# JubSteven/POEM-v2

Hardware: AMD Instinct MI355X
Metric: samples/sec (multi-view frames) POEM-medium 8-view (higher is better)
Workload: dtype f32

## Files before the change

poem-v2_amd/csrc/decoder.cpp:

```cpp
#include "engine.h"

int build_anchor_tables(poem_handle_t h, Plan& p, hipStream_t s, bool at_create) {
  const poem_config_t& c = h->cfg;
  const int C = c.embed, Q = c.nquery;
  const bool ov = !at_create && h->overlap && h->bps_stream && h->knn_stream;
  hipStream_t sk = ov ? h->knn_stream : s;
  if (ov) {
    HIPCHK(hipEventRecord(h->ev_fork0, s));
    HIPCHK(hipStreamWaitEvent(sk, h->ev_fork0, 0));
  }
  const int bb0 = h->block_base(0);
  HIPCHK(poem_launch_canon_xyz(h->tmpl, p.canon_xyz, Q * 3, c.radius, sk));
  for (int k = 0; k < 2; ++k) {
    const int vb = bb0 + (k == 0 ? B_VS : B_VC);
    HIPCHK(poem_launch_vector_attention_tables(p.canon_xyz, h->anchor, h->anchor_idx, h->R(vb + 4), h->R(vb + 5),
                                               h->P(vb + 6), h->R(vb + 7), h->fused[0].w[5 + k], p.tab_g[k], p.tab_p[k],
                                               Q, C, sk));
  }
  if (ov) HIPCHK(hipEventRecord(h->ev_tab, sk));
  h->tables_pending = ov;
  return POEM_OK;
}

namespace {
// ... 212 lines not shown
      hidden = p.h_cross[i];
      ldh = C;
      if (tables && i == 0 && !anchor_from_y3) return anchor_rows_f3(i);
      return POEM_OK;
    }
    for (int a = 0; a < 2; ++a) {
      const int ab = bb + (a == 0 ? B_A1 : B_A2);
      float* hout = a == 0 ? p.h_attn : p.h_cross[i];
      const float* qptr = p.qeqp + C;
      int ldq = 2 * C;
      if (a == 1) {
        const int rc = gemm(hidden, ldh, ab + 0, ab + 1, nullptr, 0, p.qp, C, BQ, C, C, POEM_ACT_NONE);
        if (rc != POEM_OK) return rc;
        qptr = p.qp;
        ldq = C;
      }
      if (ov && a == 0) HIPCHK(hipStreamWaitEvent(s, h->ev_bps[i], 0));
      if (h->precision == POEM_PRECISION_SPLIT_F16X3_ALL) poem_cross_attention_split(h->kv_presplit[i] ? 2 : 1);
      if (h->precision == POEM_PRECISION_FP32 && merge_in_attention() && poem_cross_attention_merges(S, C, c.heads))
        HIPCHK(poem_launch_cross_attention_merged(qptr, ldq, Q, p.y1[i] + (size_t)(2 * a) * BSP * C, p.y1[i] + (size_t)(2 * a + 1) * BSP * C,
                                                  p.ctx, B, Q, S, C, c.heads, s));
      else
        HIPCHK(poem_launch_cross_attention_img(qptr, ldq, p.y1[i] + (size_t)(2 * a) * BSP * C, p.y1[i] + (size_t)(2 * a + 1) * BSP * C,
                                               p.ctx, B, Q, S, C, c.heads, p.attn_scratch, s));
      const int rc = gemm(p.ctx, C, ab + 6, ab + 7, hidden, ldh, p.att, C, BQ, C, C, POEM_ACT_NONE);
      if (rc != POEM_OK) return rc;
      HIPCHK(poem_launch_layernorm(p.att, h->R(ab + 8), h->R(ab + 9), hout, BQ, C, c.ln_eps, s));
      hidden = hout;
      ldh = C;
    }
    if (tables && i == 0) {
      HIPCHK(poem_launch_gemm(hidden, C, h->fused[i].w[2], h->fused[i].b[2], nullptr, 0, p.y3, 3 * C, BQ, C, C, POEM_ACT_NONE, s));
      return anchor_rows_f3(i);
    }
    HIPCHK(poem_launch_gemm_split(hidden, C, h->fused[i].w[2], h->fused[i].b[2], nullptr, 0, p.y3, 3 * C, BQ, 3 * C, C, POEM_ACT_NONE,
                                  3 * C, POEM_ACT_NONE, s));
    return POEM_OK;
  }

  int vector_self(int i) {
    const int vsb = h->block_base(i) + B_VS;
    const float* xyz = p.xyz[i];
    if (ov && i > 0 && !knn_waited[i]) HIPCHK(hipStreamWaitEvent(s, h->ev_knn[i], 0));
    const bool prof = prof_begin();
    const int kq = shared ? 32 : (h->knn_query ? h->knn_query : c.knn);
    if (h->precision != POEM_PRECISION_FP32) {
      if (kq != 32) return POEM_E_UNSUPPORTED;
      const auto& sw = h->split[2 * i];
      HIPCHK(poem_launch_vector_attention_split(xyz, xyz, anchor, idx_s, shared, p.y3, p.y3 + C, p.y3 + 2 * C, Q, h->R(vsb + 4),
                                                h->R(vsb + 5), sw.w[0], h->R(vsb + 7), sw.w[1], sw.w[2], sw.scales, p.rs, B, Q, C,
                                                3 * C, 3 * C, 3 * C, s));
    } else if (tables && i == 0) {
      if (ov && h->tables_pending) HIPCHK(hipStreamWaitEvent(s, h->ev_tab, 0));
      if (anchor_from_y3)
        HIPCHK(poem_launch_vector_attention_anchored(h->anchor_idx, p.y3, p.y3 + C, p.y3 + 2 * C, Q, h->P(vsb + 10), p.tab_g[0], p.tab_p[0],
                                                     p.rs, B, Q, C, 3 * C, 3 * C, 3 * C, s));
      else {
      if (ov) HIPCHK(hipStreamWaitEvent(s, h->ev_xyz[0], 0));
      HIPCHK(poem_launch_vector_attention_anchored(p.ident, p.y3, p.anch_kv[0], p.anch_kv[0] + C, 32, h->P(vsb + 10), p.tab_g[0],
                                                   p.tab_p[0], p.rs, B, Q, C, 3 * C, 2 * C, 2 * C, s));
      }
    } else if (!shared && p.idx_ld != 32) {
      HIPCHK(poem_launch_vector_attention_k(xyz, xyz, idx_s, kq, p.idx_ld, p.y3, p.y3 + C, p.y3 + 2 * C, Q, h->R(vsb + 4), h->R(vsb + 5),
                                            h->P(vsb + 6), h->R(vsb + 7), h->fused[i].w[5], h->R(vsb + 9), h->P(vsb + 10), h->R(vsb + 11),
                                            p.rs, B, Q, C, 3 * C, 3 * C, 3 * C, 1, s));
    } else {
      poem_vecattn_one_query_blocks(h->va_p1);
      poem_vecattn_valid_neighbours(kq);
      const hipError_t ve = poem_launch_vector_attention(xyz, xyz, anchor, idx_s, shared, p.y3, p.y3 + C, p.y3 + 2 * C, Q, h->R(vsb + 4),
                                                         h->R(vsb + 5), h->P(vsb + 6), h->R(vsb + 7), h->fused[i].w[5], h->R(vsb + 9),
                                                         h->P(vsb + 10), h->R(vsb + 11), p.rs, B, Q, C, 3 * C, 3 * C, 3 * C, 1, s);
      poem_vecattn_valid_neighbours(32);
      poem_vecattn_one_query_blocks(0);
      HIPCHK(ve);
    }
    if (const int rc = prof_end(prof, tables && i == 0 ? 1 : 0); rc != POEM_OK) return rc;
    if (chain) {
      ChainArgs cc = chain_args(1);
      cc.x = p.rs; cc.ldx = C;
      cc.w1 = (const float4*)h->P(vsb + 2); cc.b1 = h->R(vsb + 3); cc.res = hidden; cc.ldres = C; cc.res_mod = 0;
      cc.y1 = p.f_self[i]; cc.ldy1 = C;
      cc.w2 = (const float4*)h->fused[i].w[4]; cc.b2 = h->fused[i].b[4]; cc.n2 = 1; cc.y2 = p.qc; cc.ldy2 = C;
      HIPCHK(poem_launch_chain(&cc, C, s));
      return POEM_OK;
    }
    if (const int rc = gemm(p.rs, C, vsb + 2, vsb + 3, hidden, C, p.f_self[i], C, BQ, C, C, POEM_ACT_NONE); rc != POEM_OK) return rc;
    HIPCHK(poem_launch_gemm(p.f_self[i], C, h->fused[i].w[4], h->fused[i].b[4], nullptr, 0, p.qc, C, BQ, C, C, POEM_ACT_NONE, s));
    return POEM_OK;
  }

  int vector_cross(int i) {
    const int vcb = h->block_base(i) + B_VC;
    const float* xyz = p.xyz[i];
    if (ov && (wmask & 2) && i == 0 && defer_at() == 0)
      for (int k = 1; k < c.nblocks; ++k) {
        HIPCHK(hipStreamWaitEvent(s, h->ev_bps[k], 0));
        bps_waited[k] = true;
      }
    const bool prof = prof_begin();
    const int kc = shared ? 32 : c.knn;
    if (h->precision != POEM_PRECISION_FP32) {
      if (kc != 32) return POEM_E_UNSUPPORTED;
      const auto& sw = h->split[2 * i + 1];
      HIPCHK(poem_launch_vector_attention_split(xyz, pt_xyz_rows, anchor, idx_c, shared, p.qc, p.y1[i] + 4 * (size_t)BSP * C,
                                                p.y1[i] + 5 * (size_t)BSP * C, SP, h->R(vcb + 4), h->R(vcb + 5), sw.w[0],
                                                h->R(vcb + 7), sw.w[1], sw.w[2], sw.scales, p.rc, B, Q, C, C, C, C, s));
    } else if (tables && i == 0) {
      if (ov) HIPCHK(hipStreamWaitEvent(s, h->ev_xyz[0], 0));
      HIPCHK(poem_launch_vector_attention_anchored(p.ident, p.qc, p.anch_kv[1], p.anch_kv[1] + C, 32, h->P(vcb + 10), p.tab_g[1],
                                                   p.tab_p[1], p.rc, B, Q, C, C, 2 * C, 2 * C, s));
    } else if (!shared && p.idx_ld != 32) {
      HIPCHK(poem_launch_vector_attention_k(xyz, pt_xyz_rows, idx_c, kc, p.idx_ld, p.qc, p.y1[i] + 4 * (size_t)BSP * C, p.y1[i] + 5 * (size_t)BSP * C,
                                            SP, h->R(vcb + 4), h->R(vcb + 5), h->P(vcb + 6), h->R(vcb + 7), h->fused[i].w[6], h->R(vcb + 9),
                                            h->P(vcb + 10), h->R(vcb + 11), p.rc, B, Q, C, C, C, C, 1, s));
    } else {
      poem_vecattn_one_query_blocks(h->va_p1);
      poem_vecattn_valid_neighbours(kc);
      const hipError_t ve = poem_launch_vector_attention(xyz, pt_xyz_rows, anchor, idx_c, shared, p.qc, p.y1[i] + 4 * (size_t)BSP * C,
                                                         p.y1[i] + 5 * (size_t)BSP * C, SP, h->R(vcb + 4), h->R(vcb + 5), h->P(vcb + 6),
                                                         h->R(vcb + 7), h->fused[i].w[6], h->R(vcb + 9), h->P(vcb + 10), h->R(vcb + 11), p.rc, B,
                                                         Q, C, C, C, C, 1, s);
      poem_vecattn_valid_neighbours(32);
      poem_vecattn_one_query_blocks(0);
      HIPCHK(ve);
    }
    return prof_end(prof, tables && i == 0 ? 1 : 0);
  }

  int parametric_tail(int i) {
    const int bb = h->block_base(i);
    HIPCHK(poem_launch_q3_flatten(feats, h->R(bb + B_FLAT_W), h->R(bb + B_FLAT_B), p.q3t, B, Q, C, s));
    HIPCHK(poem_launch_narrow_linear(p.q3t, C, h->R(bb + B_MANO_W), h->R(bb + B_MANO_B), nullptr, p.par, B, C, 106, s));
    HIPCHK(poem_launch_rot6d_to_aa(p.par, pose_aa, betas, B, s));
    if (h->mano_table) HIPCHK(poem_launch_mano_lbs(pose_aa, betas, h->mano_table, p.mano_verts, p.mano_joints, B, h->mano_center, s));
    return POEM_OK;
  }

  int tail(int i, bool* done) {
    const int bb = h->block_base(i), vcb = bb + B_VC;
    const float* xyz = p.xyz[i];
    const bool last = i == c.nblocks - 1;
    const bool feats_dead = last && !c.parametric && !h->taps;
    *done = feats_dead;
    if (chain) {
      ChainArgs cd = chain_args(2);
      cd.x = p.rc; cd.ldx = C;
      cd.w1 = (const float4*)h->P(vcb + 2); cd.b1 = h->R(vcb + 3); cd.res = p.f_self[i]; cd.ldres = C; cd.res_mod = 0;
      cd.y1 = p.f_cross[i]; cd.ldy1 = C;
      cd.wf4 = (const float4*)h->fused[i].w[3]; cd.bf4 = h->fused[i].b[3];
      cd.wreg2 = h->R(bb + B_REG2_W); cd.breg2 = h->R(bb + B_REG2_B); cd.xyz_in = xyz; cd.xyz_out = p.xyz[i + 1];
      HIPCHK(poem_launch_chain(&cd, C, s));
      if (feats_dead) return POEM_OK;
      const bool early = ov && h->knn_early && !last;
      const bool d2_first = early && h->d2_first != 0;
      if (early && d2_first) HIPCHK(hipEventRecord(h->ev_xyz[i + 1], s));
      if (early && !d2_first)
        if (const int rc = neighbour_searches(i + 1); rc != POEM_OK) return rc;
      ChainArgs ce = chain_args(3);
      ce.x = p.f_cross[i]; ce.ldx = C;
      ce.wf4 = (const float4*)h->fused[i].w[3]; ce.bf4 = h->fused[i].b[3];
      ce.wout = (const float4*)h->P(bb + B_OUT_W); ce.bout = h->R(bb + B_OUT_B);
      ce.ln2_g = h->R(bb + B_LN_W); ce.ln2_b = h->R(bb + B_LN_B); ce.y3 = p.feats[i]; ce.ldy3 = C;
      if (!last) {
// ... 67 lines not shown
```

poem-v2_amd/csrc/engine.h:

```cpp
#pragma once
#include "../../include/poem_hip.h"
#include "launchers.h"

#include <hip/hip_runtime.h>

#include <algorithm>
#include <cstdio>
#include <cstdlib>
#include <cstring>
#include <map>
#include <string>
#include <vector>

extern thread_local int g_last_hip_error;

#define HIPCHK(expr)                                 \
  do {                                               \
    (void)hipGetLastError();                         \
    hipError_t e_ = (expr);                          \
    if (e_ != hipSuccess) {                          \
      g_last_hip_error = (int)e_;                    \
      return POEM_E_LAUNCH;                          \
    }                                                \
  } while (0)
// ... 48 lines not shown
  std::vector<SplitW> split;
  void* split_mem = nullptr;
  int precision = 0;
  bool kv_presplit[8] = {};
  const char* packed_base = nullptr;
  size_t packed_size = 0;
  char* native16 = nullptr;
  char* gemm_split = nullptr;
  float* gemm_scales = nullptr;
  bool taps = false;
  struct Tap { const void* p; int64_t elems; };
  std::map<std::string, Tap> tapmap;
  std::vector<hipEvent_t> prof_ev;
  int prof_used = 0;
  std::vector<char> prof_kind;
  bool prof_on = false;
  hipStream_t bps_stream = nullptr, knn_stream = nullptr;
  hipEvent_t ev_fork = nullptr, ev_join_bps = nullptr, ev_join_knn = nullptr, ev_tab = nullptr, ev_fork0 = nullptr;
  bool anchor_tables = true;
  bool chains = true;
  bool fused_sampling = true;
  bool tables_first = true;
  bool chain_combine = true;
  int xattn_merge = -1;
  bool knn_early = true;
  bool graphs = true;
  bool graph_broken = false;
  hipStream_t cap_stream = nullptr;
  int stream_device = 0;
  struct GraphEntry { std::vector<int64_t> key; hipGraphExec_t exec; uint64_t stamp; uint64_t shape; hipStream_t last_stream = nullptr; bool launched = false; };
  std::vector<GraphEntry> graph_cache;
  std::vector<std::vector<int64_t>> graph_seen;
  bool graph_eager = false;
  uint64_t graph_clock = 0;
  static constexpr size_t GRAPH_CAP = 12;
  int64_t graph_captures = 0, graph_instantiations = 0, graph_replays = 0, plain_forwards = 0, layout_uploads = 0;
  int small_batch = 3;
  int group_xcd = 1;
  int group_min_views = 0;
  const float* mano_table = nullptr;
  int mano_center = 9;
  int knn_query = 0;
  int knn_fma = 0;
  int chain_tile = 0;
  bool tables_cached = true;
  bool tables_pending = false;
  float* tab_mem = nullptr;
  float *c_canon_xyz = nullptr, *c_tab_g[2] = {}, *c_tab_p[2] = {};
  float* c_qeqp0 = nullptr;
  hipEvent_t ev_bps[8] = {}, ev_xyz[8] = {}, ev_knn[8] = {}, ev_def[8] = {};
  int bps_defer = 0;
  bool f1_split = true;
  int va_p1 = -1;
  int d2_first = 1;
  int wait_merge = -1;
  bool overlap = true;
  static constexpr int IDX_CAP = 32768;
  int32_t* idx_dev = nullptr;
  std::vector<int32_t> idx_host;
  int block_base(int b) const { return T_HEAD_COUNT + b * (cfg.parametric ? B_COUNT_PARAM : B_COUNT); }
  const float* R(int idx) const { return raw[idx]; }
  const void* P(int idx) const { return packed[idx]; }
};

struct Arena {
  char* base;
  size_t off = 0;
  explicit Arena(void* b) : base((char*)b) {}
  template <typename T>
  T* take(size_t n) {
    off = align_up(off, 256);
    T* p = base ? (T*)(base + off) : nullptr;
    off += n * sizeof(T);
    return p;
  }
};

struct Plan {
  int32_t *offs, *view_sample, *pe_index, *idx_self[8], *idx_cross[8];
  float *x, *uv, *g, *h1, *h2, *mm, *mh, *y, *bps_feat, *centre, *pt_xyz, *xyz[9];
  float *xt, *ptab, *q1;
  float *petr_f, *petr_h, *petr_tab;
  float *feats0, *qp, *ctx, *att, *h_attn, *y3, *rs, *qc, *rc, *y4, *ffo;
  float *y1[8];
  float *qeqp;
  float *h_cross[8], *f_self[8], *f_cross[8], *feats[8];
  float *q3t, *par, *attn_scratch, *g_pose, *g_betas;
  float *mano_verts, *mano_joints;
  float *canon_xyz, *tab_g[2], *tab_p[2];
  float *anch_x[2], *anch_kv[2], *qeqp0;
  int32_t* ident;
  float *feat_pad, *xyz_pad;
  int idx_ld;
  size_t bytes;
};

inline int padded_samples(const poem_config_t& c) { return (c.nsample + 31) / 32 * 32; }

inline int neighbour_ld(const poem_config_t& c, int knn_query) { return (c.knn > 32 || knn_query > 32) ? 64 : 32; }

Plan make_plan(const poem_config_t& c, int B, int BN, void* base, int idx_ld);
void register_taps(poem_handle_t h, const Plan& p, int B, int BN, bool sampling);

int poem_process_switches();
void poem_park_graph_exec(hipGraphExec_t e, uint64_t shape, int device, hipStream_t last_stream, bool launched);
hipGraphExec_t poem_reuse_graph_exec(hipGraph_t graph, uint64_t shape, int device);
// ... 5 lines not shown
```

poem-v2_amd/csrc/forward.cpp:

```cpp
#include "engine.h"

namespace {

struct SplitContext {
  bool set = false;
  explicit SplitContext(poem_handle_t h) {
    if (h->precision != POEM_PRECISION_SPLIT_F16X3_ALL) return;
    set = true;
    poem_gemm_split_context(h->packed_base, h->packed_size, h->gemm_split, h->gemm_scales);
    poem_cross_attention_split(1);
    const int dh = h->cfg.embed / h->cfg.heads;
    poem_gemm_split_images(dh == 32 || dh == 64);
  }
  ~SplitContext() {
    if (!set) return;
    poem_gemm_split_context(nullptr, 0, nullptr, nullptr);
    poem_cross_attention_split(0);
    poem_gemm_split_images(0);
  }
};

struct HeadRun {
  poem_handle_t h;
  const poem_config_t& c;
// ... 106 lines not shown
      SampleMergeArgs sm{};
      sm.xt = p.xt; sm.tab = (const float4*)p.ptab; sm.tabo = (const uint2*)(p.ptab + (size_t)plan_views * S * 4);
      sm.view_sample = p.view_sample; sm.offs = p.offs;
      sm.w0 = (const float4*)h->P(T_M00_W); sm.b0 = h->R(T_M00_B); sm.w1 = (const float4*)h->P(T_M02_W); sm.b1 = h->R(T_M02_B);
      sm.h2 = p.h2; sm.q1 = p.q1; sm.S = S; sm.hw = HW; sm.h2_tiled = 1;
      sm.views = plan_views; sm.B = B; sm.views_dev = p.offs + B;
      const bool group_ok = h->group_min_views >= 0 && (S / C) % 8 == 0;
      sm.group_min_views = group_ok ? (h->group_min_views > 0 ? h->group_min_views : 2 * poem_device_cu_count() / ((C / (C == 512 ? 32 : 64)) * (S / C / 8)))
                                    : 0x7fffffff;
      if (h->tables_first && h->tables_pending) HIPCHK(hipStreamWaitEvent(st, h->ev_tab, 0));
      MergeTailArgs mt{};
      mt.h2 = p.h2; mt.q1 = p.q1; mt.offs = p.offs;
      mt.w0 = (const float4*)h->P(T_M10_W); mt.b0 = h->R(T_M10_B); mt.w1 = (const float4*)h->P(T_M12_W); mt.b1 = h->R(T_M12_B);
      mt.out = p.bps_feat; mt.B = B; mt.S = S; mt.h2_tiled = 1;
      mt.group_min_views = sm.group_min_views; mt.views_dev = sm.views_dev; mt.views = sm.views;
      sm.xcd_order = h->group_xcd;
      if (group_ok && plan_views >= sm.group_min_views) {
        SampleGroupArgs sg{};
        sg.sm = sm; sg.w2 = mt.w0; sg.b2 = mt.b0; sg.w3 = mt.w1; sg.b3 = mt.b1; sg.out = p.bps_feat;
        HIPCHK(poem_launch_sample_group(&sg, C, st));
      }
      HIPCHK(poem_launch_sample_merge(&sm, C, st));
      HIPCHK(poem_launch_merge_tail(&mt, C, st));
      return POEM_OK;
    }
    auto gemm = [&](const float* X, int ldx, int wi, int bi, float* Y, int ldy, int M, int N, int K, int act) -> int {
      HIPCHK(poem_launch_gemm(X, ldx, h->P(wi), h->R(bi), nullptr, 0, Y, ldy, M, N, K, act, st));
      return POEM_OK;
    };
    HIPCHK(poem_launch_grid_sample(p.x, p.uv, p.g, BN, C, c.feat_h, c.feat_w, S, st));
    int rc = gemm(p.g, C, T_M00_W, T_M00_B, p.h1, C, BN * S, C, C, POEM_ACT_RELU);
    if (rc == POEM_OK) rc = gemm(p.h1, C, T_M02_W, T_M02_B, p.h2, C / 2, BN * S, C / 2, C, POEM_ACT_NONE);
    if (rc != POEM_OK) return rc;
    HIPCHK(poem_launch_merge_reduce(p.h2, p.offs, p.mm, B, S, C / 2, st));
    rc = gemm(p.mm, C / 2, T_M10_W, T_M10_B, p.mh, C / 2, BS, C / 2, C / 2, POEM_ACT_RELU);
    if (rc == POEM_OK) rc = gemm(p.mh, C / 2, T_M12_W, T_M12_B, p.y, C, BS, C, C / 2, POEM_ACT_NONE);
    if (rc != POEM_OK) return rc;
    HIPCHK(poem_launch_merge_finalize(p.g, p.y, p.offs, p.bps_feat, B, S, C, st));
    return POEM_OK;
  }

  int body(hipStream_t st, float* pose_dst, float* betas_dst) {
    if (const int rc = sampling(st); rc != POEM_OK) return rc;
    if (prof_fe) HIPCHK(hipEventRecord(h->prof_ev[2 * prof_slot + 1], st));
    if (!(h->anchor_tables && h->precision == POEM_PRECISION_FP32 && (h->small_batch & 1)))
      HIPCHK(poem_launch_broadcast(h->R(T_QEMB), p.feats0, (long)Q * C, B, st));
    return run_decoder(h, p, p.feats0, p.pt_xyz, p.bps_feat, B, pose_dst, betas_dst, st, true);
  }

  int replay(void* workspace, float* pose_aa, float* betas) {
    if (!h->graphs || h->graph_broken || h->prof_on || h->tables_pending || !h->cap_stream) return 0;
    const std::vector<int64_t> key = {B, plan_views, fused_fe ? -1 : BN, (int64_t)(uintptr_t)workspace, h->precision, h->anchor_tables, h->chains,
                                      h->fused_sampling, h->tables_first, h->chain_combine, h->knn_early, h->overlap, h->chain_tile,
                                      h->tables_cached, h->knn_fma, h->knn_query, h->taps, c.parametric, h->xattn_merge, h->small_batch, h->bps_defer, poem_process_switches(), h->f1_split, h->va_p1, h->group_min_views, h->group_xcd, h->d2_first, h->wait_merge,
                                      (int64_t)(uintptr_t)h->mano_table, h->mano_center};
    poem_handle_s::GraphEntry* hit = nullptr;
    for (auto& g : h->graph_cache)
      if (g.key == key) { hit = &g; break; }
    if (!hit) {
      if (!h->graph_eager) {
        bool seen = false;
        for (auto& k : h->graph_seen) seen = seen || k == key;
        if (!seen) {
          if (h->graph_seen.size() >= 64) h->graph_seen.erase(h->graph_seen.begin());
          h->graph_seen.push_back(key);
          return 0;
        }
      }
      hipGraph_t graph = nullptr;
      hipGraphExec_t exec = nullptr;
      POEM_TRACE("capture begin h=%p B=%d cached=%zu", (void*)h, B, h->graph_cache.size());
      bool ok = hipStreamBeginCapture(h->cap_stream, hipStreamCaptureModeRelaxed) == hipSuccess;
      if (ok) {
        const int rc = body(h->cap_stream, p.g_pose, p.g_betas);
        POEM_TRACE("capture body rc=%d", rc);
        const hipError_t e = hipStreamEndCapture(h->cap_stream, &graph);
        POEM_TRACE("capture end e=%d graph=%p", (int)e, (void*)graph);
        ok = rc == POEM_OK && e == hipSuccess && graph != nullptr;
      }
      ++h->graph_captures;
      if (ok) {
        exec = poem_reuse_graph_exec(graph, graph_shape_of(c, key), h->stream_device);
        if (!exec) {
          ok = hipGraphInstantiate(&exec, graph, nullptr, nullptr, 0) == hipSuccess;
          ++h->graph_instantiations;
        }
      }
      POEM_TRACE("instantiate ok=%d exec=%p", (int)ok, (void*)exec);
      if (graph) (void)hipGraphDestroy(graph);
      POEM_TRACE("graph destroyed");
      if (!ok) {
        (void)hipGetLastError();
        h->graph_broken = true;
        return 0;
      }
      if (h->graph_cache.size() >= poem_handle_s::GRAPH_CAP) {
        size_t lru = 0;
        for (size_t i = 1; i < h->graph_cache.size(); ++i)
          if (h->graph_cache[i].stamp < h->graph_cache[lru].stamp) lru = i;
        poem_park_graph_exec(h->graph_cache[lru].exec, h->graph_cache[lru].shape, h->stream_device, h->graph_cache[lru].last_stream,
                             h->graph_cache[lru].launched);
        h->graph_cache.erase(h->graph_cache.begin() + lru);
      }
      h->graph_cache.push_back({key, exec, 0, graph_shape_of(c, key), nullptr, false});
      hit = &h->graph_cache.back();
    }
    hit->stamp = ++h->graph_clock;
// ... 101 lines not shown
```

poem-v2_amd/csrc/handle.cpp:

```cpp
#include "engine.h"

#include <atomic>
thread_local int g_last_hip_error = 0;

static std::atomic<int> g_proc_switches{15};
int poem_process_switches() { return g_proc_switches.load(); }

#include <mutex>
namespace {
struct CaptureKit {
  hipStream_t cap = nullptr, bps = nullptr, knn = nullptr;
  hipEvent_t ev[5 + 32] = {};
};
std::mutex g_pool_mutex;
std::map<int, std::vector<CaptureKit>> g_kit_pool;
struct ParkedExec { hipGraphExec_t exec; uint64_t shape; int device; hipEvent_t done; };
std::vector<ParkedExec> g_parked_execs;
std::map<int, std::vector<hipEvent_t>> g_idle_done_events;
int64_t g_exec_reuses = 0, g_exec_update_failures = 0, g_exec_busy_skips = 0;

hipEvent_t done_event_locked(hipStream_t last_stream, bool launched, int device, bool* ok) {
  *ok = true;
  if (!launched) return nullptr;
  int cur = -1;
// ... 431 lines not shown
void poem_destroy(poem_handle_t h) {
  if (!h) return;
  POEM_TRACE("destroy h=%p graphs=%zu", (void*)h, h->graph_cache.size());
  for (auto e : h->prof_ev) (void)hipEventDestroy(e);
  if (h->tab_mem) (void)hipFree(h->tab_mem);
  if (h->split_mem) (void)hipFree(h->split_mem);
  if (h->gemm_split) (void)hipFree(h->gemm_split);
  if (h->native16) (void)hipFree(h->native16);
  if (h->gemm_scales) (void)hipFree(h->gemm_scales);
  park_execs(h);
  return_kit(h);
  delete h;
}

int poem_set_overlap(poem_handle_t h, int enable) {
  if (!h) return POEM_E_ARG;
  h->overlap = enable != 0;
  return POEM_OK;
}

int poem_set_chains(poem_handle_t h, int enable) {
  if (!h) return POEM_E_ARG;
  h->chains = enable != 0;
  return POEM_OK;
}

int poem_set_option(poem_handle_t h, const char* name, int value) {
  if (!h || !name) return POEM_E_ARG;
  const std::string k(name);
  if (k == "overlap") h->overlap = value != 0;
  else if (k == "anchor_tables") h->anchor_tables = value != 0;
  else if (k == "chains") h->chains = value != 0;
  else if (k == "knn_early") h->knn_early = value != 0;
  else if (k == "fused_sampling") h->fused_sampling = value != 0;
  else if (k == "chain_combine") h->chain_combine = value != 0;
  else if (k == "xattn_merge") { if (value < -1 || value > 1) return POEM_E_ARG; h->xattn_merge = value; }
  else if (k == "tables_first") h->tables_first = value != 0;
  else if (k == "tables_cached") h->tables_cached = value != 0;
  else if (k == "knn_fma") h->knn_fma = value != 0;
  else if (k == "knn_query") {
    if (value < 0 || value > 64 || value > h->cfg.nquery) return POEM_E_ARG;
    if (h->precision != POEM_PRECISION_FP32 && value != 0 && value != 32) return POEM_E_UNSUPPORTED;
    h->knn_query = value;
  }
  else if (k == "graphs") h->graphs = value != 0;
  else if (k == "graph_eager") h->graph_eager = value != 0;
  else if (k == "gemm_xcd_map") { poem_gemm_xcd_map(value != 0); g_proc_switches.fetch_and(~1); g_proc_switches.fetch_or(value ? 1 : 0); }
  else if (k == "f1_split") h->f1_split = value != 0;
  else if (k == "xattn_half") { poem_cross_attention_half(value != 0); g_proc_switches.fetch_and(~4); g_proc_switches.fetch_or(value ? 4 : 0); }
  else if (k == "xattn_tail") { poem_cross_attention_tail_halves(value != 0); g_proc_switches.fetch_and(~8); g_proc_switches.fetch_or(value ? 8 : 0); }
  else if (k == "wait_merge") { if (value < -1 || value > 7) return POEM_E_ARG; h->wait_merge = value; }
  else if (k == "d2_first") { if (value < 0 || value > 1) return POEM_E_ARG; h->d2_first = value; }
  else if (k == "va_p1") { if (value < -1 || value > 2) return POEM_E_ARG; h->va_p1 = value; }
  else if (k == "gemm_kslab") { poem_gemm_kslab(value != 0); g_proc_switches.fetch_and(~2); g_proc_switches.fetch_or(value ? 2 : 0); }
  else if (k == "small_batch") h->small_batch = value;
  else if (k == "group_xcd") h->group_xcd = value != 0;
  else if (k == "group_min_views") { if (value < -1) return POEM_E_ARG; h->group_min_views = value; }
  else if (k == "bps_defer") { if (value < 0 || value > 3) return POEM_E_ARG; h->bps_defer = value; }
  else if (k == "chain_tile") { if (value < 0 || value > 3) return POEM_E_ARG; h->chain_tile = value; }
  else return POEM_E_ARG;
  return POEM_OK;
}

int poem_graph_stats(poem_handle_t h, int64_t* out, int n) {
  if (!h || !out || n < 9) return POEM_E_ARG;
  out[0] = (int64_t)h->graph_cache.size();
  out[1] = h->graph_captures; out[2] = h->graph_instantiations; out[3] = h->graph_replays; out[4] = h->plain_forwards;
  out[5] = h->layout_uploads;
  std::lock_guard<std::mutex> lock(g_pool_mutex);
  out[6] = (int64_t)g_parked_execs.size(); out[7] = g_exec_reuses; out[8] = g_exec_update_failures;
  if (n >= 10) out[9] = g_exec_busy_skips;
  return POEM_OK;
}

int poem_attach_mano(poem_handle_t h, const void* table, int center_idx) {
  if (!h || center_idx < -1 || center_idx > 20) return POEM_E_ARG;
  if (table && !h->cfg.parametric) return POEM_E_UNSUPPORTED;
  h->mano_table = (const float*)table;
  h->mano_center = center_idx;
  return POEM_OK;
}

int poem_set_anchor_tables(poem_handle_t h, int enable) {
  if (!h) return POEM_E_ARG;
  h->anchor_tables = enable != 0;
  return POEM_OK;
}

int poem_set_precision(poem_handle_t h, int mode) {
  if (!h || mode < POEM_PRECISION_FP32 || mode > POEM_PRECISION_SPLIT_F16X3_ALL) return POEM_E_ARG;
  if (mode != POEM_PRECISION_FP32 && (!h->split_mem || !h->gemm_split)) return POEM_E_UNSUPPORTED;
  if (mode != POEM_PRECISION_FP32 && (h->cfg.knn != 32 || (h->knn_query && h->knn_query != 32)))
    return POEM_E_UNSUPPORTED;
  if (mode != POEM_PRECISION_FP32 && h->cfg.nsample % 32)
    return POEM_E_UNSUPPORTED;
  h->precision = mode;
  return POEM_OK;
}

int poem_enable_taps(poem_handle_t h, int enable) {
  if (!h) return POEM_E_ARG;
  h->taps = enable != 0;
  return POEM_OK;
}

int64_t poem_tap(poem_handle_t h, const char* name, void* dst, int64_t dst_elems, void* stream) {
// ... 58 lines not shown
```

poem-v2_amd/csrc/launchers.h:

```cpp
#pragma once
#include <hip/hip_runtime.h>

#include "../../include/poem_hip.h"
#include "chain.h"
#include "conv.h"
#include "loss.h"
#include "merge.h"

extern "C" {
hipError_t poem_launch_pack_linear(const float* w, int N, int K, void* out, hipStream_t s);
hipError_t poem_launch_gemm(const float* X, int ldx, const void* Wp, const float* bias, const float* R, int ldr,
                            float* Y, int ldy, int M, int N, int K, int act, hipStream_t s);
hipError_t poem_launch_gemm2(const float* X, int ldx, const void* Wp, const float* bias, const float* R, int ldr,
                             float* Y, int ldy, int M, int N, int K, int act, int in_pa, int out_pa, hipStream_t s);
hipError_t poem_launch_unpack_rows(const void* pa, int N, int K, float* out, hipStream_t s);
hipError_t poem_launch_layernorm(const float* x, const float* g, const float* b, float* y, int rows, int cols,
                                 float eps, hipStream_t s);
hipError_t poem_launch_narrow_linear(const float* x, int ldx, const float* w, const float* b, const float* base,
                                     float* out, int rows, int K, int N, hipStream_t s);
hipError_t poem_launch_sine_pe(float* out, int F, int H, int W, int max_views, int normalize, hipStream_t s);
hipError_t poem_launch_frustum_features(const float* intr, const float* extr, float* out, int views, int H, int W, int D, int lid,
                                        double depth_start, double depth_end, const double* position_range, int img0, int img1,
                                        hipStream_t s);
hipError_t poem_launch_conv1x1_ex(const float* feat, const void* Wp, const float* bias, const float* table, const int* pe_index,
// ... 35 lines not shown
hipError_t poem_launch_cross_attention_imgq(const float* q, int ldq, int q_batch_rows, const void* kimg, const void* vimg,
                                            float* ctx, int B, int NQ, int NK, int C, int heads, float* scratch, hipStream_t s);
int poem_chain_supported(int C);
int poem_chain_combines(int C, int heads, int chunks);
void poem_cross_attention_partials(int B, int NQ, int NK, int C, int heads, float* scratch, const void** part_o,
                                   const void** part_ml, int* chunks, float* kc2);
hipError_t poem_launch_chain(const ChainArgs* a, int C, hipStream_t s);
hipError_t poem_launch_native16(const void* packed, void* native, size_t bytes, hipStream_t s);
int poem_chain16_wants_native(int C);
hipError_t poem_launch_knn(const float* qxyz, const float* sxyz, int* idx, int B, int NQ, int NS, int fma, hipStream_t s);
hipError_t poem_launch_knn_k(const float* qxyz, const float* sxyz, int* idx, int B, int NQ, int NS, int K, int ld, int fma,
                             hipStream_t s);
hipError_t poem_launch_vector_attention(const float* query_xyz, const float* src_xyz, const float* anchor_xyz,
                                        const int* idx, int shared_idx, const float* q, const float* k, const float* v,
                                        int nsrc, const float* wd1, const float* bd1, const void* wd2, const float* bd2,
                                        const void* wg1, const float* bg1, const void* wg2, const float* bg2, float* out,
                                        int B, int Q, int C, int ldq, int ldk, int ldv, int composed, hipStream_t s);
hipError_t poem_launch_vector_attention_k(const float* query_xyz, const float* src_xyz, const int* idx, int K, int ld,
                                          const float* q, const float* k, const float* v, int nsrc, const float* wd1,
                                          const float* bd1, const void* wd2, const float* bd2, const void* wg1, const float* bg1,
                                          const void* wg2, const float* bg2, float* out, int B, int Q, int C, int ldq, int ldk,
                                          int ldv, int composed, hipStream_t s);
size_t poem_vector_attention_table_floats(int Q, int C);
hipError_t poem_launch_vector_attention_tables(const float* query_xyz, const float* anchor_xyz, const int* idx,
                                               const float* wd1, const float* bd1, const void* wd2, const float* bd2,
                                               const void* wg1d2, float* tab_g, float* tab_p, int Q, int C, hipStream_t s);
hipError_t poem_launch_vector_attention_anchored(const int* idx, const float* qg, const float* kg, const float* v, int nsrc,
                                                 const void* wg2, const float* tab_g, const float* tab_p, float* out, int B,
                                                 int Q, int C, int ldq, int ldk, int ldv, hipStream_t s);
hipError_t poem_launch_gather_anchor_rows(const float* src, int ld, const int* idx, int NS, float* dst, int B, int C,
                                          int* ident, hipStream_t s);
hipError_t poem_launch_pad_rows(const float* src, float* dst, int B, int S, int SP, int W, hipStream_t s);
hipError_t poem_launch_canon_xyz(const float* tmpl, float* out, int n, float radius, hipStream_t s);
hipError_t poem_launch_pack_split(const float* w, int C, void* img, float* scale_out, hipStream_t s);
hipError_t poem_launch_pack_split_tiles(const float* w, int N, int K, void* img, float* scales, int scale_stride, hipStream_t s);
void poem_gemm_split_context(const void* packed, size_t bytes, const void* split, const float* scales);
void poem_gemm_split_explicit(const void* img, const float* scales);
void poem_cross_attention_split(int on);
void poem_cross_attention_masked_form(int on);
void poem_cross_attention_half(int on);
void poem_cross_attention_tail_halves(int on);
int poem_cross_attention_merges(int NK, int C, int heads);
int poem_cross_attention_fits(int B, int NK, int C);
hipError_t poem_launch_cross_attention_merged_rm(const float* q, const float* k, const float* v, float* ctx, int B, int NQ, int NK,
                                                 int C, int heads, float* scratch, hipStream_t s);
hipError_t poem_launch_cross_attention_merged(const float* q, int ldq, int q_batch_rows, const void* kimg, const void* vimg, float* ctx,
                                              int B, int NQ, int NK, int C, int heads, hipStream_t s);
int poem_gemm_split_applies(const void* Wp, int M, int ldx, int K);
void poem_gemm_split_images(int on);
void poem_gemm_xcd_map(int on);
void poem_gemm_kslab(int on);
void poem_vecattn_one_query_blocks(int on);
void poem_vecattn_valid_neighbours(int k);
hipError_t poem_launch_vector_attention_split(const float* query_xyz, const float* src_xyz, const float* anchor_xyz,
                                              const int* idx, int shared_idx, const float* q, const float* k,
                                              const float* v, int nsrc, const float* wd1, const float* bd1,
                                              const void* wd2, const float* bd2, const void* wg1, const void* wg2,
                                              const float* scales, float* out, int B, int Q, int C, int ldq,
                                              int ldk, int ldv, hipStream_t s);
hipError_t poem_launch_dlt(const float* uv, const float* intr, const float* mat, const int* offs, float* out, int B, int J,
                           int invert, hipStream_t s);
hipError_t poem_launch_dlt_confidence(const float* uv, const float* conf, const float* intr, const float* mat,
                                      const int* offs, float* out, int* sel_count, int B, int J, int invert, int mode,
                                      double threshold, hipStream_t s);
hipError_t poem_launch_dlt_robust(const float* uv, const float* intr, const float* mat, const int* offs, float* out,
                                  unsigned char* inlier, int* count, float* resid, int B, int J, int invert,
                                  double inlier_px, int refine, hipStream_t s);
hipError_t poem_launch_pa_epe(const float* pred, const float* gt, float* out, int B, int P, hipStream_t s);
hipError_t poem_launch_pck_accumulate(const float* pred, const float* gt, int B, int P, double vmin, double vmax, int steps,
                                      unsigned int* counts, double* sum, unsigned int* n, float* dist_out, hipStream_t s);
hipError_t poem_launch_pa_align(const float* pred, const float* gt, float* aligned, double* transform, int B, int P, hipStream_t s);
size_t poem_nn_distance_slots(int B, int na, int nb);
hipError_t poem_launch_nn_distance(const float* a, int na, const float* b, int nb, float* dist_ab, float* dist_ba,
                                   const double* thr, int nthr, int* counts, double* sums, void* workspace, int B, hipStream_t s);
hipError_t poem_launch_mano_to_openpose(const float* jreg, const float* verts, float* joints, int B, int nverts,
                                        hipStream_t s);
hipError_t poem_launch_warp_affine(const unsigned char* src, const long long* src_off, const int* src_hw,
                                   const double* minv, const double* gain, float* out_f32, unsigned char* out_u8, int views,
                                   int OH, int OW, hipStream_t s);
hipError_t poem_launch_jpeg_reconstruct(const poem_jpeg_desc_t* descs, const int16_t* coef, long long coef_bytes,
                                        const long long* out_offsets, unsigned char* out, long long out_bytes, int n,
                                        long long total_blocks, long long total_quads, unsigned char* planes, hipStream_t s);
extern "C" size_t poem_jpeg_entropy_ws_bytes(int n, long long total_subs);
extern "C" hipError_t poem_launch_jpeg_entropy(poem_jpeg_desc_t* descs, const poem_jpeg_scan_t* scans, const poem_jpeg_huff_t* tables,
                                               long long table_count, const unsigned char* packed, long long packed_bytes, int n, int subseq,
                                               int wg_threads, long long total_subs, long long total_blocks, int16_t* coef,
                                               long long coef_bytes, int* status, void* workspace, hipStream_t s);
hipError_t poem_launch_heatmap_uv(const float* hmap, float* uv, int maps, int hh, int hw, float img_w, float img_h,
                                  hipStream_t s);
hipError_t poem_launch_heatmap_uv_conf(const float* hmap, float* uv, float* conf, int maps, int hh, int hw, float img_w,
                                       float img_h, hipStream_t s);
size_t poem_conv3x3_packed_floats(int Cout, int Cin);
hipError_t poem_launch_upcat_conv3x3(const float* a_half, int Ca, const float* b_full, int Cb, const void* wp, const float* scale,
                                     const float* shift, float* out, int views, int Cout, int H, int W, int relu, ConvMap omap,
                                     hipStream_t s);
hipError_t poem_launch_pack_conv3x3(const float* w, int Cout, int Cin, void* out, hipStream_t s);
hipError_t poem_launch_conv3x3(const float* in, const void* wp, const float* scale, const float* shift, const float* res,
                               float* out, int views, int Cin, int Cout, int H, int W, int stride, int relu, ConvMap omap,
                               hipStream_t s);
hipError_t poem_launch_conv3x3_ex(const float* in, const void* wp, const float* scale, const float* shift, const float* res,
                                  ConvMap rmap, int res_pre, float* out, int views, int Cin, int Cout, int H, int W, int stride,
                                  int relu, ConvMap omap, hipStream_t s);
size_t poem_conv1x1_packed_floats(int Cout, int Cin);
hipError_t poem_launch_pack_conv1x1(const float* w, int Cout, int Cin, void* out, hipStream_t s);
hipError_t poem_launch_conv1x1_nchw(const Conv1Args* a, hipStream_t s);
hipError_t poem_launch_hrnet_fuse(const FuseArgs* a, hipStream_t s);
// ... 58 lines not shown
```

poem-v2_amd/csrc/vecattn.hip:

```cpp
#include "common.h"
#ifndef POEM_VA_XCD_SAMPLES
#define POEM_VA_XCD_SAMPLES 1
#endif
#include <algorithm>
#include <cstdlib>

#ifdef POEM_VA_DBG
__device__ long long va_dbg[64 * 4 * 8];
#define VA_STAMP(k) do { if (item >= 6000 && item < 6064 && lane == 0) va_dbg[((item - 6000) * 4 + wv) * 8 + (k)] = clock64(); } while (0)
#else
#define VA_STAMP(k) do { } while (0)
#endif

struct VecAttnArgs {
  const float* query_xyz;
  const float* src_xyz;
  const float* anchor_xyz;
  const int* idx;
  int shared_idx;
  const float* q;
  const float* k;
  const float* v;
  int NS;
  const float* wd1;
// ... 422 lines not shown
#pragma unroll
      for (int i = 0; i < 16; ++i) pt[i] = COMP ? pos[tp][p][i] : scr[mfma_row(i, h) * 33 + j];
      f32x16& a = acc[tp][p];
      if (MASK) {
#pragma unroll
        for (int i = 0; i < 16; ++i)
          if (mfma_row(i, h) >= A.kvalid) a[i] = -INFINITY;
      }
      if (WIDE) {
#pragma unroll
        for (int i = 0; i < 16; ++i)
          if (32 * ch + mfma_row(i, h) >= A.kvalid) a[i] = -INFINITY;
      }
      float mx = fmaxf(fmaxf(a[0], a[1]), a[2]);
#pragma unroll
      for (int i = 3; i < 15; i += 2) mx = fmaxf(fmaxf(mx, a[i]), a[i + 1]);
      mx = half_max(fmaxf(mx, a[15]));
      const float nb = -mx * k2;
      const f32x2 k2v = {k2, k2}, nbv = {nb, nb};
      f32x2 sum2 = {0.f, 0.f}, res2 = {0.f, 0.f};
      asm volatile("s_waitcnt lgkmcnt(0)" ::: "memory");
#pragma unroll
      for (int i = 0; i < 16; i += 2) {
        f32x2 e = __builtin_elementwise_fma(f32x2{a[i], a[i + 1]}, k2v, nbv);
        e[0] = __builtin_amdgcn_exp2f(e[0]);
        e[1] = __builtin_amdgcn_exp2f(e[1]);
        const f32x2 val = f32x2{vg[i], vg[i + 1]} + f32x2{pt[i], pt[i + 1]};
        sum2 += e;
        res2 = __builtin_elementwise_fma(e, val, res2);
      }
      const float sum = half_sum(sum2[0] + sum2[1]);
      const float res = half_sum(res2[0] + res2[1]);
      if (WIDE) {
        if (ch == 0) {
          wmx[q] = mx; wsum[q] = sum; wres[q] = res;
        } else {
          const float m = fmaxf(wmx[q], mx), nm = -m * k2;
          const float so = __builtin_amdgcn_exp2f(__builtin_fmaf(wmx[q], k2, nm)), sn = __builtin_amdgcn_exp2f(__builtin_fmaf(mx, k2, nm));
          wsum[q] = __builtin_fmaf(wsum[q], so, sum * sn);
          wres[q] = __builtin_fmaf(wres[q], so, res * sn);
          wmx[q] = m;
        }
        if (ch == nch - 1 && h == 0 && i0 + p < A.Q) A.out[((size_t)b * A.Q + i0 + p) * C + cch] = wres[q] * __builtin_amdgcn_rcpf(wsum[q]);
      } else if (h == 0 && i0 + p < A.Q) A.out[((size_t)b * A.Q + i0 + p) * C + cch] = res * __builtin_amdgcn_rcpf(sum);
    }
  }
  if constexpr (WIDE)
    if (++ch < nch) goto va_chunk;
#undef VA_GATHER
  VA_STAMP(7);
  }
}

template <int C, int P, int NW, int MINW, bool COMP, int MODE = 0>
static hipError_t launch_va_t(const VecAttnArgs& a, hipStream_t s) {
  const int groups = (a.Q + P - 1) / P;
  size_t lds = (size_t)C * 32 * P * 4 + P * 32 * 3 * 4 + 2 * P * 32 * 4 + (size_t)P * C * 4;
#ifdef POEM_VA_DBG
  if (const char* e = getenv("POEM_VA_LDSPAD")) lds += atoi(e);
#endif
  auto kern = vecattn_kernel<C, P, NW, MINW, COMP, MODE>;
  static std::atomic<unsigned long long> optin{0};
  if (hipError_t e = poem_optin_lds(reinterpret_cast<const void*>(kern), lds, optin); e != hipSuccess) return e;
  unsigned grid = (unsigned)(a.B * groups);
  if (a.stagger > 0) {
    grid = std::min(grid, (unsigned)(2 * poem_device_cus()));
  }
  hipLaunchKernelGGL(kern, dim3(grid), dim3(NW * 64), lds, s, a);
  return hipGetLastError();
}

template <int C, int P, int NW, int MINW>
static hipError_t launch_va(const VecAttnArgs& a, hipStream_t s, int mode = 0) {
  if (mode == 4) return a.composed ? launch_va_t<C, P, NW, MINW, true, 4>(a, s) : launch_va_t<C, P, NW, MINW, false, 4>(a, s);
  if (mode == 1) return launch_va_t<C, P, NW, MINW, true, 1>(a, s);
  if (mode == 2) return launch_va_t<C, P, NW, MINW, true, 2>(a, s);
  if (mode == 3) return a.composed ? launch_va_t<C, P, NW, MINW, true, 3>(a, s) : hipErrorInvalidValue;
  return a.composed ? launch_va_t<C, P, NW, MINW, true>(a, s) : launch_va_t<C, P, NW, MINW, false>(a, s);
}

static thread_local int g_va_kvalid = 32;
extern "C" void poem_vecattn_valid_neighbours(int k) { g_va_kvalid = k; }

static thread_local int g_va_p1 = 0;
extern "C" void poem_vecattn_one_query_blocks(int on) { g_va_p1 = on; }

static int va_group_size(int C) { return C == 128 ? 4 : (C >= 512 ? 1 : 2); }

static hipError_t dispatch_va(const VecAttnArgs& a, int C, hipStream_t s, int mode) {
  if (mode != 1 && (unsigned long long)a.NS * a.ldv * 4 + (unsigned long long)C * 4 > (1ull << 31)) return hipErrorInvalidValue;
  if (mode == 4 && (a.kvalid < 1 || a.kvalid > 64 || a.ldidx < a.kvalid || a.shared_idx || a.anchor_xyz)) return hipErrorInvalidValue;
  if (mode == 0 && a.kvalid != 32) {
    if (a.kvalid < 1 || a.kvalid > 32) return hipErrorInvalidValue;
    mode = 3;
  }
  switch (C) {
    case 32: return launch_va<32, 2, 1, 1>(a, s, mode);
    case 64: return launch_va<64, 2, 2, 1>(a, s, mode);
    case 128: return launch_va<128, 4, 4, 2>(a, s, mode);
    case 256: {
      const int g_va_p1 = ::g_va_p1 >= 0 ? ::g_va_p1 : ((long)a.B * a.Q <= 16L * poem_device_cus() ? 1 : 0);
      if (mode == 0 && g_va_p1 == 1 && a.composed) return launch_va_t<256, 1, 4, 3, true>(a, s);
      if (mode == 0 && g_va_p1 == 2 && a.composed) return launch_va_t<256, 1, 4, 2, true>(a, s);
      return launch_va<256, 2, 4, 2>(a, s, mode);
    }
    case 512: return launch_va<512, 1, 4, 2>(a, s, mode);
    case 1024: return launch_va<1024, 1, 8, 2>(a, s, mode);
    default: return hipErrorInvalidValue;
  }
}

extern "C" size_t poem_vector_attention_table_floats(int Q, int C) {
  const int P = va_group_size(C);
  return (size_t)((Q + P - 1) / P) * P * 32 * C;
}

extern "C" hipError_t poem_launch_vector_attention_tables(const float* query_xyz, const float* anchor_xyz, const int* idx,
                                                          const float* wd1, const float* bd1, const void* wd2,
                                                          const float* bd2, const void* wg1d2, float* tab_g,
                                                          float* tab_p, int Q, int C, hipStream_t s) {
  VecAttnArgs a{query_xyz, nullptr, anchor_xyz, idx, 1, nullptr, nullptr, nullptr, 1, wd1, bd1, (const float4*)wd2, bd2,
                (const float4*)wg1d2, nullptr, nullptr, nullptr, nullptr, 1, Q, 0, 0, 0, 0, 1, (float4*)tab_g, (float4*)tab_p, 32, 32};
  return dispatch_va(a, C, s, 1);
}

extern "C" hipError_t poem_launch_vector_attention_anchored(const int* idx, const float* qg, const float* kg,
                                                            const float* v, int nsrc, const void* wg2,
                                                            const float* tab_g, const float* tab_p, float* out, int B,
                                                            int Q, int C, int ldq, int ldk, int ldv, hipStream_t s) {
// ... 43 lines not shown
```

Baseline: 1470.

## Add persistent walk kernel for anchored vector attention reusing position tables

After: 1476 (median of 6 runs). No clear change (+0.4%).

```diff
diff --git a/poem-v2_amd/csrc/decoder.cpp b/poem-v2_amd/csrc/decoder.cpp
--- a/poem-v2_amd/csrc/decoder.cpp
+++ b/poem-v2_amd/csrc/decoder.cpp
@@ -288,14 +288,15 @@
                                                 3 * C, 3 * C, 3 * C, s));
     } else if (tables && i == 0) {
       if (ov && h->tables_pending) HIPCHK(hipStreamWaitEvent(s, h->ev_tab, 0));
-      if (anchor_from_y3)
-        HIPCHK(poem_launch_vector_attention_anchored(h->anchor_idx, p.y3, p.y3 + C, p.y3 + 2 * C, Q, h->P(vsb + 10), p.tab_g[0], p.tab_p[0],
-                                                     p.rs, B, Q, C, 3 * C, 3 * C, 3 * C, s));
-      else {
-      if (ov) HIPCHK(hipStreamWaitEvent(s, h->ev_xyz[0], 0));
-      HIPCHK(poem_launch_vector_attention_anchored(p.ident, p.y3, p.anch_kv[0], p.anch_kv[0] + C, 32, h->P(vsb + 10), p.tab_g[0],
-                                                   p.tab_p[0], p.rs, B, Q, C, 3 * C, 2 * C, 2 * C, s));
-      }
+      if (!anchor_from_y3 && ov) HIPCHK(hipStreamWaitEvent(s, h->ev_xyz[0], 0));
+      poem_vecattn_anchored_walk(h->va_anchor_walk);
+      const hipError_t ve = anchor_from_y3
+          ? poem_launch_vector_attention_anchored(h->anchor_idx, p.y3, p.y3 + C, p.y3 + 2 * C, Q, h->P(vsb + 10), p.tab_g[0], p.tab_p[0],
+                                                  p.rs, B, Q, C, 3 * C, 3 * C, 3 * C, s)
+          : poem_launch_vector_attention_anchored(p.ident, p.y3, p.anch_kv[0], p.anch_kv[0] + C, 32, h->P(vsb + 10), p.tab_g[0],
+                                                  p.tab_p[0], p.rs, B, Q, C, 3 * C, 2 * C, 2 * C, s);
+      poem_vecattn_anchored_walk(0);
+      HIPCHK(ve);
     } else if (!shared && p.idx_ld != 32) {
       HIPCHK(poem_launch_vector_attention_k(xyz, xyz, idx_s, kq, p.idx_ld, p.y3, p.y3 + C, p.y3 + 2 * C, Q, h->R(vsb + 4), h->R(vsb + 5),
                                             h->P(vsb + 6), h->R(vsb + 7), h->fused[i].w[5], h->R(vsb + 9), h->P(vsb + 10), h->R(vsb + 11),
@@ -343,8 +344,11 @@
                                                 h->R(vcb + 7), sw.w[1], sw.w[2], sw.scales, p.rc, B, Q, C, C, C, C, s));
     } else if (tables && i == 0) {
       if (ov) HIPCHK(hipStreamWaitEvent(s, h->ev_xyz[0], 0));
-      HIPCHK(poem_launch_vector_attention_anchored(p.ident, p.qc, p.anch_kv[1], p.anch_kv[1] + C, 32, h->P(vcb + 10), p.tab_g[1],
-                                                   p.tab_p[1], p.rc, B, Q, C, C, 2 * C, 2 * C, s));
+      poem_vecattn_anchored_walk(h->va_anchor_walk);
+      const hipError_t ve = poem_launch_vector_attention_anchored(p.ident, p.qc, p.anch_kv[1], p.anch_kv[1] + C, 32, h->P(vcb + 10), p.tab_g[1],
+                                                                  p.tab_p[1], p.rc, B, Q, C, C, 2 * C, 2 * C, s);
+      poem_vecattn_anchored_walk(0);
+      HIPCHK(ve);
     } else if (!shared && p.idx_ld != 32) {
       HIPCHK(poem_launch_vector_attention_k(xyz, pt_xyz_rows, idx_c, kc, p.idx_ld, p.qc, p.y1[i] + 4 * (size_t)BSP * C, p.y1[i] + 5 * (size_t)BSP * C,
                                             SP, h->R(vcb + 4), h->R(vcb + 5), h->P(vcb + 6), h->R(vcb + 7), h->fused[i].w[6], h->R(vcb + 9),
diff --git a/poem-v2_amd/csrc/engine.h b/poem-v2_amd/csrc/engine.h
--- a/poem-v2_amd/csrc/engine.h
+++ b/poem-v2_amd/csrc/engine.h
@@ -124,6 +124,7 @@
   int bps_defer = 0;
   bool f1_split = true;
   int va_p1 = -1;
+  int va_anchor_walk = -1;
   int d2_first = 1;
   int wait_merge = -1;
   bool overlap = true;
diff --git a/poem-v2_amd/csrc/forward.cpp b/poem-v2_amd/csrc/forward.cpp
--- a/poem-v2_amd/csrc/forward.cpp
+++ b/poem-v2_amd/csrc/forward.cpp
@@ -182,7 +182,7 @@
     if (!h->graphs || h->graph_broken || h->prof_on || h->tables_pending || !h->cap_stream) return 0;
     const std::vector<int64_t> key = {B, plan_views, fused_fe ? -1 : BN, (int64_t)(uintptr_t)workspace, h->precision, h->anchor_tables, h->chains,
                                       h->fused_sampling, h->tables_first, h->chain_combine, h->knn_early, h->overlap, h->chain_tile,
-                                      h->tables_cached, h->knn_fma, h->knn_query, h->taps, c.parametric, h->xattn_merge, h->small_batch, h->bps_defer, poem_process_switches(), h->f1_split, h->va_p1, h->group_min_views, h->group_xcd, h->d2_first, h->wait_merge,
+                                      h->tables_cached, h->knn_fma, h->knn_query, h->taps, c.parametric, h->xattn_merge, h->small_batch, h->bps_defer, poem_process_switches(), h->f1_split, h->va_p1, h->va_anchor_walk, h->group_min_views, h->group_xcd, h->d2_first, h->wait_merge,
                                       (int64_t)(uintptr_t)h->mano_table, h->mano_center};
     poem_handle_s::GraphEntry* hit = nullptr;
     for (auto& g : h->graph_cache)
diff --git a/poem-v2_amd/csrc/handle.cpp b/poem-v2_amd/csrc/handle.cpp
--- a/poem-v2_amd/csrc/handle.cpp
+++ b/poem-v2_amd/csrc/handle.cpp
@@ -507,6 +507,7 @@
   else if (k == "wait_merge") { if (value < -1 || value > 7) return POEM_E_ARG; h->wait_merge = value; }
   else if (k == "d2_first") { if (value < 0 || value > 1) return POEM_E_ARG; h->d2_first = value; }
   else if (k == "va_p1") { if (value < -1 || value > 2) return POEM_E_ARG; h->va_p1 = value; }
+  else if (k == "va_anchor_walk") { if (value < -1 || value > 65536) return POEM_E_ARG; h->va_anchor_walk = value; }
   else if (k == "gemm_kslab") { poem_gemm_kslab(value != 0); g_proc_switches.fetch_and(~2); g_proc_switches.fetch_or(value ? 2 : 0); }
   else if (k == "small_batch") h->small_batch = value;
   else if (k == "group_xcd") h->group_xcd = value != 0;
diff --git a/poem-v2_amd/csrc/launchers.h b/poem-v2_amd/csrc/launchers.h
--- a/poem-v2_amd/csrc/launchers.h
+++ b/poem-v2_amd/csrc/launchers.h
@@ -111,6 +111,7 @@
 void poem_gemm_kslab(int on);
 void poem_vecattn_one_query_blocks(int on);
 void poem_vecattn_valid_neighbours(int k);
+void poem_vecattn_anchored_walk(int blocks);
 hipError_t poem_launch_vector_attention_split(const float* query_xyz, const float* src_xyz, const float* anchor_xyz,
                                               const int* idx, int shared_idx, const float* q, const float* k,
                                               const float* v, int nsrc, const float* wd1, const float* bd1,
diff --git a/poem-v2_amd/csrc/vecattn.hip b/poem-v2_amd/csrc/vecattn.hip
--- a/poem-v2_amd/csrc/vecattn.hip
+++ b/poem-v2_amd/csrc/vecattn.hip
@@ -498,6 +498,173 @@
   }
 }
 
+template <int C, int P, int NW, int MINW, int GT>
+__global__ __launch_bounds__(NW * 64, MINW) void vecattn_walk_kernel(VecAttnArgs A) {
+  constexpr int NTILE = C / 32;
+  constexpr int TPW = C / 32 / NW;
+  constexpr int XS = 32 * P;
+  constexpr int NT = NW * 64;
+  static_assert(GT >= 0 && GT <= TPW, "resident tab_g tiles: at most the wave's own");
+  extern __shared__ __attribute__((aligned(16))) float smem[];
+  float* X = smem;
+  int* voffs = reinterpret_cast<int*>(smem + C * XS + P * 32 * 3) + P * 32;
+  float* qs = reinterpret_cast<float*>(voffs + P * 32);
+
+  const int tid = threadIdx.x, lane = tid & 63, wv = tid >> 6, j = lane & 31, h = lane >> 5;
+  const int groups = (A.Q + P - 1) / P;
+  const int total = A.B * groups;
+  const float inv_sqrt_c = 1.0f / sqrtf((float)C);
+
+  const int nblk = (int)gridDim.x;
+  int slot = (int)blockIdx.x;
+  if ((nblk & 7) == 0) slot = (slot & 7) * (nblk >> 3) + (slot >> 3);
+  const int base = total / nblk, rem = total % nblk;
+  int item = slot * base + min(slot, rem);
+  const int end = item + base + (slot < rem ? 1 : 0);
+  if (item >= end) return;
+
+  if (tid < 32 * P) voffs[tid] = (int)((unsigned)A.idx[tid & 31] * (unsigned)(A.ldv * 4));
+  const int kid = A.idx[j];
+
+  f32x16 acc[TPW][P], pos[TPW][P];
+  float4 gf[TPW][P][4];
+  int ig_res = -1;
+
+  for (; item < end; ++item) {
+  const int ig = item / A.B, b = item - ig * A.B;
+  const int i0 = ig * P;
+
+  for (int f = tid; f < P * C / 4; f += NT) {
+    const int p = f / (C / 4), c4 = f % (C / 4);
+    const int qi = min(i0 + p, A.Q - 1);
+    reinterpret_cast<float4*>(qs)[f] = *reinterpret_cast<const float4*>(A.q + ((size_t)b * A.Q + qi) * A.ldq + 4 * c4);
+  }
+  float4 kgr[TPW][4];
+#pragma unroll
+  for (int tp = 0; tp < TPW; ++tp) {
+    const int cbase = (wv * TPW + tp) * 32 + 4 * h;
+    const float* krow = A.k + ((size_t)b * A.NS + kid) * A.ldk + cbase;
+#pragma unroll
+    for (int g = 0; g < 4; ++g) kgr[tp][g] = *reinterpret_cast<const float4*>(krow + 8 * g);
+  }
+  __builtin_amdgcn_sched_barrier(0);
+
+  const float4* tg = A.tab_g + ((size_t)ig * NTILE + wv * TPW) * (P * 4 * 64) + lane;
+#pragma unroll
+  for (int tp = GT; tp < TPW; ++tp)
+#pragma unroll
+    for (int p = 0; p < P; ++p)
+#pragma unroll
+      for (int g = 0; g < 4; ++g) gf[tp][p][g] = tg[((tp * P + p) * 4 + g) * 64];
+  if (ig != ig_res) {
+#pragma unroll
+    for (int tp = 0; tp < GT; ++tp)
+#pragma unroll
+      for (int p = 0; p < P; ++p)
+#pragma unroll
+        for (int g = 0; g < 4; ++g) gf[tp][p][g] = tg[((tp * P + p) * 4 + g) * 64];
+    const float4* tq = A.tab_p + ((size_t)ig * NTILE + wv * TPW) * (P * 4 * 64) + lane;
+#pragma unroll
+    for (int tp = 0; tp < TPW; ++tp)
+#pragma unroll
+      for (int p = 0; p < P; ++p)
+#pragma unroll
+        for (int g = 0; g < 4; ++g) {
+          const float4 t = tq[((tp * P + p) * 4 + g) * 64];
+#pragma unroll
+          for (int e = 0; e < 4; ++e) pos[tp][p][4 * g + e] = (&t.x)[e];
+        }
+    ig_res = ig;
+  }
+  __syncthreads();
+
+#pragma unroll
+  for (int tp = 0; tp < TPW; ++tp) {
+    const int cbase = (wv * TPW + tp) * 32 + 4 * h;
+#pragma unroll
+    for (int g = 0; g < 4; ++g)
+#pragma unroll
+      for (int p = 0; p < P; ++p) {
+        const float4 qq = *reinterpret_cast<const float4*>(qs + p * C + cbase + 8 * g);
+#pragma unroll
+        for (int e = 0; e < 4; e += 2) {
+          const int i = 4 * g + e;
+          const f32x2 tv = (f32x2{(&qq.x)[e], (&qq.x)[e + 1]} - f32x2{(&kgr[tp][g].x)[e], (&kgr[tp][g].x)[e + 1]}) +
+                           f32x2{(&gf[tp][p][g].x)[e], (&gf[tp][p][g].x)[e + 1]};
+          X[((wv * TPW + tp) * 32 + mfma_row(i, h)) * XS + 32 * p + j] = fmaxf(tv[0], 0.f);
+          X[((wv * TPW + tp) * 32 + mfma_row(i + 1, h)) * XS + 32 * p + j] = fmaxf(tv[1], 0.f);
+        }
+      }
+  }
+  __syncthreads();
+
+  chain_gemm<C, P, NW, TPW, true>(A.wg2, X, acc, wv, lane);
+
+  const float k2 = inv_sqrt_c * 1.44269504088896340736f;
+  const __amdgpu_buffer_rsrc_t vrs = frag_rsrc(A.v + (size_t)b * A.NS * A.ldv, 0xffffffffu);
+  float vgb[2][16];
+#define VA_GATHER(Q)                                                                                          \
+  {                                                                                                           \
+    const int tp_ = (Q) / P, p_ = (Q) % P, cch_ = (wv * TPW + tp_) * 32 + j;                                  \
+    _Pragma("unroll") for (int i = 0; i < 16; ++i)                                                            \
+      vgb[(Q) & 1][i] = __builtin_bit_cast(float, __builtin_amdgcn_raw_buffer_load_b32(vrs, voffs[p_ * 32 + mfma_row(i, h)] + cch_ * 4, 0, 0)); \
+  }
+  VA_GATHER(0)
+#pragma unroll
+  for (int q = 0; q < TPW * P; ++q) {
+    const int tp = q / P, p = q % P;
+    const int cch = (wv * TPW + tp) * 32 + j;
+    {
+      if (q + 1 < TPW * P) VA_GATHER(q + 1)
+      __builtin_amdgcn_sched_barrier(0);
+      const float (&vg)[16] = vgb[q & 1];
+      asm volatile("s_waitcnt lgkmcnt(0)" ::: "memory");
+      float pt[16];
+#pragma unroll
+      for (int i = 0; i < 16; ++i) pt[i] = pos[tp][p][i];
+      f32x16& a = acc[tp][p];
+      float mx = fmaxf(fmaxf(a[0], a[1]), a[2]);
+#pragma unroll
+      for (int i = 3; i < 15; i += 2) mx = fmaxf(fmaxf(mx, a[i]), a[i + 1]);
+      mx = half_max(fmaxf(mx, a[15]));
+      const float nb = -mx * k2;
+      const f32x2 k2v = {k2, k2}, nbv = {nb, nb};
+      f32x2 sum2 = {0.f, 0.f}, res2 = {0.f, 0.f};
+      asm volatile("s_waitcnt lgkmcnt(0)" ::: "memory");
+#pragma unroll
+      for (int i = 0; i < 16; i += 2) {
+        f32x2 e = __builtin_elementwise_fma(f32x2{a[i], a[i + 1]}, k2v, nbv);
+        e[0] = __builtin_amdgcn_exp2f(e[0]);
+        e[1] = __builtin_amdgcn_exp2f(e[1]);
+        const f32x2 val = f32x2{vg[i], vg[i + 1]} + f32x2{pt[i], pt[i + 1]};
+        sum2 += e;
+        res2 = __builtin_elementwise_fma(e, val, res2);
+      }
+      const float sum = half_sum(sum2[0] + sum2[1]);
+      const float res = half_sum(res2[0] + res2[1]);
+      if (h == 0 && i0 + p < A.Q) A.out[((size_t)b * A.Q + i0 + p) * C + cch] = res * __builtin_amdgcn_rcpf(sum);
+    }
+  }
+#undef VA_GATHER
+  }
+}
+
+static constexpr int va_walk_resident(int C) { return C >= 512 ? 3 : 1; }
+static thread_local int g_va_walk = 0;
+extern "C" void poem_vecattn_anchored_walk(int blocks) { g_va_walk = blocks; }
+
+template <int C, int P, int NW, int MINW, int GT>
+static hipError_t launch_va_walk(const VecAttnArgs& a, hipStream_t s, int blocks) {
+  const int groups = (a.Q + P - 1) / P;
+  const size_t lds = (size_t)C * 32 * P * 4 + P * 32 * 3 * 4 + 2 * P * 32 * 4 + (size_t)P * C * 4;
+  auto kern = vecattn_walk_kernel<C, P, NW, MINW, GT>;
+  static std::atomic<unsigned long long> optin{0};
+  if (hipError_t e = poem_optin_lds(reinterpret_cast<const void*>(kern), lds, optin); e != hipSuccess) return e;
+  const unsigned grid = blocks > 0 ? (unsigned)blocks : std::min((unsigned)(a.B * groups), (unsigned)(2 * poem_device_cus()));
+  hipLaunchKernelGGL(kern, dim3(grid), dim3(NW * 64), lds, s, a);
+  return hipGetLastError();
+}
+
 template <int C, int P, int NW, int MINW, bool COMP, int MODE = 0>
 static hipError_t launch_va_t(const VecAttnArgs& a, hipStream_t s) {
   const int groups = (a.Q + P - 1) / P;
@@ -520,7 +687,7 @@
 static hipError_t launch_va(const VecAttnArgs& a, hipStream_t s, int mode = 0) {
   if (mode == 4) return a.composed ? launch_va_t<C, P, NW, MINW, true, 4>(a, s) : launch_va_t<C, P, NW, MINW, false, 4>(a, s);
   if (mode == 1) return launch_va_t<C, P, NW, MINW, true, 1>(a, s);
-  if (mode == 2) return launch_va_t<C, P, NW, MINW, true, 2>(a, s);
+  if (mode == 2) return g_va_walk != 0 ? launch_va_walk<C, P, NW, MINW, va_walk_resident(C)>(a, s, g_va_walk) : launch_va_t<C, P, NW, MINW, true, 2>(a, s);
   if (mode == 3) return a.composed ? launch_va_t<C, P, NW, MINW, true, 3>(a, s) : hipErrorInvalidValue;
   return a.composed ? launch_va_t<C, P, NW, MINW, true>(a, s) : launch_va_t<C, P, NW, MINW, false>(a, s);
 }
```
